# volume-em/empanada-napari

Measured on AMD Instinct MI355X. Metric: EM tiles/sec (1024^2 fp16), higher is better.
Workload: dtype f16

## Files before the change

### empanada-napari_amd/build.py

```python
import os
import shutil
import subprocess
import sys

HERE = os.path.dirname(os.path.abspath(__file__))
CSRC = os.path.join(HERE, 'csrc')
OBJ = os.path.join(CSRC, '_obj')
LIBDIR = os.path.join(HERE, 'lib')
LIB = os.path.join(LIBDIR, 'libempanada_hip.so')
ARCH = 'gfx950'

COMMON = ['--offload-arch=' + ARCH, '-O3', '-std=c++17', '-fPIC', '-fvisibility=hidden',
          '-Wall', '-Wno-unused-function', '-Wno-unused-result']
PER_FILE = {
    'postprocess.hip': ['-ffp-contract=off', '-fhip-fp32-correctly-rounded-divide-sqrt'],
    'pdl_net.hip': ['-std=c++20'],
    'pdl_net32.hip': ['-std=c++20'],
}
SOURCES = ['abi.hip', 'conv_igemm.hip', 'layers.hip', 'pointrend.hip', 'postprocess.hip', 'pdl_net.hip', 'pdl_net32.hip', 'sparse.hip',
           'sepconv.hip', 'sepconv_precise.hip', 'conv_igemm256.hip', 'conv_igemm_s64.hip', 'conv3x3c64.hip', 'stem.hip', 'matcher.hip', 'ref32.hip', 'conv16x3.hip', 'conv_igemm_grouped.hip', 'conv16x3p.hip', 'sepconv_x3.hip', 'overlap.hip', 'labels.hip', 'measure.hip', 'morph.hip', 'split.hip']
INCLUDES = {'conv_igemm_grouped.hip': ['conv_igemm.hip']}


def _hipcc():
    for cand in (shutil.which('hipcc'), '/opt/rocm/bin/hipcc'):
        if cand and os.path.exists(cand):
            return cand
    raise RuntimeError('hipcc not found: the HIP engine cannot be built (no CPU fallback exists)')


def _newest_header():
    hs = [os.path.join(CSRC, f) for f in os.listdir(CSRC) if f.endswith('.h')]
    hs.append(os.path.join(HERE, '..', 'include', 'empanada_hip.h'))
    return max(os.path.getmtime(h) for h in hs)


def build_all(verbose=False, force=False):
    os.makedirs(OBJ, exist_ok=True)
    os.makedirs(LIBDIR, exist_ok=True)
    hipcc = _hipcc()
    hdr = _newest_header()
    objs, rebuilt = [], False
    procs = []
    for src in SOURCES:
        s = os.path.join(CSRC, src)
        o = os.path.join(OBJ, src.replace('.hip', '.o'))
        objs.append(o)
        dep = max([os.path.getmtime(s), hdr] + [os.path.getmtime(os.path.join(CSRC, d)) for d in INCLUDES.get(src, [])])
        if force or not os.path.exists(o) or os.path.getmtime(o) < dep:
            cmd = [hipcc] + COMMON + PER_FILE.get(src, []) + ['-c', s, '-o', o]
            if verbose:
                print(' '.join(cmd), flush=True)
            procs.append((src, subprocess.Popen(cmd, stdout=subprocess.PIPE, stderr=subprocess.STDOUT)))
            rebuilt = True
    for src, p in procs:
        out, _ = p.communicate()
        if p.returncode != 0:
            sys.stderr.write(out.decode())
            raise RuntimeError(f'hipcc failed on {src}')
        if verbose and out.strip():
            print(out.decode())
    if rebuilt or not os.path.exists(LIB):
        cmd = [hipcc, '--offload-arch=' + ARCH, '-shared', '-fPIC', '-o', LIB] + objs
        if verbose:
            print(' '.join(cmd), flush=True)
        subprocess.check_call(cmd)
    return LIB


if __name__ == '__main__':
    print(build_all(verbose=True, force='--force' in sys.argv))
```

### empanada-napari_amd/csrc/abi.hip

```cpp
#include <stdarg.h>

#include <map>
#include <mutex>
#include <utility>
#include <vector>

#include "common.h"

namespace emp {

static thread_local char g_err[1024] = "no error";

void set_error(const char* fmt, ...) {
  va_list ap;
  va_start(ap, fmt);
  vsnprintf(g_err, sizeof(g_err), fmt, ap);
  va_end(ap);
}

const void* zero_page() {
  static void* page = nullptr;
  static std::once_flag once;
  std::call_once(once, [] {
    if (hipMalloc(&page, 2048) != hipSuccess) { page = nullptr; return; }
    if (hipMemset(page, 0, 2048) != hipSuccess) { (void)hipFree(page); page = nullptr; }
  });
  return page;
}

int ensure_dyn_lds(const void* kernel, int bytes) {
  static std::mutex mu;
  static std::map<std::pair<int, const void*>, int> done;
  int dev = 0;
  EMP_CHECK_HIP(hipGetDevice(&dev));
  std::lock_guard<std::mutex> lk(mu);
  auto it = done.find({dev, kernel});
  if (it != done.end() && it->second >= bytes) return EMP_OK;
  EMP_CHECK_HIP(hipFuncSetAttribute(kernel, hipFuncAttributeMaxDynamicSharedMemorySize, bytes));
  done[{dev, kernel}] = bytes;
  return EMP_OK;
}

}

using namespace emp;

extern "C" {

const char* emp_last_error(void) { return g_err; }
int emp_abi_version(void) { return 5; }

int emp_device_count(void) {
  int n = 0;
  hipError_t e = hipGetDeviceCount(&n);
  if (e != hipSuccess) {
    set_error("hipGetDeviceCount: %s", hipGetErrorString(e));
    return EMP_ERR_HIP;
  }
  return n;
}

int emp_copy_d2d(void* d_dst, const void* d_src, size_t bytes, void* stream) {
  EMP_REQUIRE(d_dst && d_src, "copy_d2d: null pointer");
  EMP_CHECK_HIP(hipMemcpyAsync(d_dst, d_src, bytes, hipMemcpyDeviceToDevice, (hipStream_t)stream));
  return EMP_OK;
}

int emp_conv2d_nhwc_f16(const void* d_in, int N, int H, int W, int Cin, int in_ld, const void* d_w,
                        const float* d_bias, const float* d_bias_n, const void* d_res, int res_ld, void* d_out,
                        int out_ld, int Cout, int KH, int KW, int stride, int pad, int dil, int relu, int variant,
                        void* stream) {
  EMP_REQUIRE(d_in && d_w && d_out, "conv2d: null pointer");
  EMP_REQUIRE(N > 0 && H > 0 && W > 0 && KH > 0 && KW > 0 && stride > 0 && dil > 0 && pad >= 0, "conv2d: bad geometry");
  EMP_REQUIRE(variant >= 0 && (variant & 15) <= 3 && ((variant >> 4) & 15) <= 7 && ((variant >> 8) & 255) <= 64 && (variant >> 16) <= 31, "conv2d: bad variant %d", variant);
  ConvParams p{};
  p.in = (const half_t*)d_in;
  p.wgt = (const half_t*)d_w;
  p.bias = d_bias;
  p.bias_n = d_bias_n;
  p.res = (const half_t*)d_res;
  p.res_ld = res_ld;
  p.out = (half_t*)d_out;
  p.zero = (const half_t*)zero_page();
  EMP_REQUIRE(p.zero != nullptr, "conv2d: could not allocate the zero page");
  p.N = N; p.H = H; p.W = W; p.Cin = Cin; p.in_ld = in_ld;
  p.Cout = Cout; p.KH = KH; p.KW = KW; p.stride = stride; p.pad = pad; p.dil = dil;
  p.Ho = (H + 2 * pad - dil * (KH - 1) - 1) / stride + 1;
  p.Wo = (W + 2 * pad - dil * (KW - 1) - 1) / stride + 1;
  EMP_REQUIRE(p.Ho > 0 && p.Wo > 0, "conv2d: empty output");
  p.out_ld = out_ld;
  p.act = relu;
  p.ps_cout = 0;
  p.M = N * p.Ho * p.Wo;
  return launch_conv_igemm(p, variant, (hipStream_t)stream);
}

int emp_conv256_pack_weights(const void* d_w, void* d_packed, int Cout, int KT, int Cin, int Cin2, void* stream) {
  return conv256_pack_weights((const half_t*)d_w, (half_t*)d_packed, Cout, KT, Cin, Cin2, (hipStream_t)stream);
}

int emp_conv2d_nhwc_f32(const float* d_in, int N, int H, int W, int Cin, int in_ld, const float* d_w, const float* d_bias,
                        const float* d_bias_n, const float* d_res, int res_ld, float* d_out, int out_ld, int Cout, int KH,
                        int KW, int stride, int pad, int dil, int act, void* stream) {
  EMP_REQUIRE(d_in && d_w && d_out, "conv2d_f32: null pointer");
  EMP_REQUIRE(N > 0 && H > 0 && W > 0 && KH > 0 && KW > 0 && stride > 0 && dil > 0 && pad >= 0, "conv2d_f32: bad geometry");
  Conv32 p{};
  p.in = d_in; p.in_ld = in_ld; p.w = d_w; p.bias = d_bias; p.bias_n = d_bias_n; p.res = d_res; p.res_ld = res_ld;
  p.out = d_out; p.out_ld = out_ld;
  p.N = N; p.H = H; p.W = W; p.Cin = Cin; p.Cout = Cout; p.KH = KH; p.KW = KW; p.stride = stride; p.pad = pad; p.dil = dil;
  p.Ho = (H + 2 * pad - dil * (KH - 1) - 1) / stride + 1;
  p.Wo = (W + 2 * pad - dil * (KW - 1) - 1) / stride + 1;
  EMP_REQUIRE(p.Ho > 0 && p.Wo > 0 && out_ld >= Cout && (d_res == nullptr || res_ld >= Cout), "conv2d_f32: bad output geometry");
  p.act = act;
  return launch_conv32(p, (hipStream_t)stream);
}

int emp_conv2d_nhwc_f16x3(const float* d_in, int N, int H, int W, int Cin, int in_ld, const float* d_w, const float* d_bias,
                          const float* d_bias_n, const float* d_res, int res_ld, float* d_out, int out_ld, int Cout, int KH,
                          int KW, int stride, int pad, int dil, int act, int groups, int cin_g, void* stream) {
  EMP_REQUIRE(d_in && d_w && d_out, "conv2d_f16x3: null pointer");
  EMP_REQUIRE(N > 0 && H > 0 && W > 0 && KH > 0 && KW > 0 && stride > 0 && dil > 0 && pad >= 0 && groups >= 1, "conv2d_f16x3: bad geometry");
  Conv32 p{};
  p.in = d_in; p.in_ld = in_ld; p.w = d_w; p.bias = d_bias; p.bias_n = d_bias_n; p.res = d_res; p.res_ld = res_ld;
  p.out = d_out; p.out_ld = out_ld;
  p.N = N; p.H = H; p.W = W; p.Cin = Cin; p.Cout = Cout; p.KH = KH; p.KW = KW; p.stride = stride; p.pad = pad; p.dil = dil;
  p.Ho = (H + 2 * pad - dil * (KH - 1) - 1) / stride + 1;
  p.Wo = (W + 2 * pad - dil * (KW - 1) - 1) / stride + 1;
  EMP_REQUIRE(p.Ho > 0 && p.Wo > 0 && out_ld >= groups * Cout && (d_res == nullptr || res_ld >= Cout), "conv2d_f16x3: bad output geometry");
  p.act = act;
  p.x3 = 1;
  if (groups > 1) { p.groups = groups; p.cin_g = cin_g; }
  return launch_conv32(p, (hipStream_t)stream);
}

int emp_conv2d_nhwc_f16x3_ex(const float* d_in, int N, int H, int W, int Cin, int in_ld, const float* d_w, const float* d_bias,
                             const float* d_bias_n, const float* d_res, int res_ld, void* d_out, int out_ld, int out_fmt, int Cout, int KH,
                             int KW, int stride, int pad, int dil, int act, int wmode, const float* d_in2, int H2, int W2, int Cin2,
                             int in2_ld, int stride2, const float* d_head_w, const float* d_head_b, int head_c, float* d_head_out,
                             void* stream) {
  EMP_REQUIRE(d_in && d_w && (d_out || d_head_w), "conv2d_f16x3_ex: null pointer");
  EMP_REQUIRE(N > 0 && H > 0 && W > 0 && KH > 0 && KW > 0 && stride > 0 && dil > 0 && pad >= 0 && wmode >= 0 && (wmode & 3) <= 2 && wmode < 8,
              "conv2d_f16x3_ex: bad geometry (wmode 0 fp32 weights, 1 split pairs, 2 pairs + LDS-DMA image; + 4: split-K allowed)");
  const bool ksplit = (wmode & 4) != 0;
  wmode &= 3;
  hipStream_t s = (hipStream_t)stream;
  Conv32 p{};
  p.in = d_in; p.in_ld = in_ld; p.w = d_w; p.bias = d_bias; p.bias_n = d_bias_n; p.res = d_res; p.res_ld = res_ld;
  p.out = (float*)d_out; p.out_ld = out_ld; p.out_fmt = out_fmt;
  p.N = N; p.H = H; p.W = W; p.Cin = Cin; p.Cout = Cout; p.KH = KH; p.KW = KW; p.stride = stride; p.pad = pad; p.dil = dil;
  p.Ho = (H + 2 * pad - dil * (KH - 1) - 1) / stride + 1;
  p.Wo = (W + 2 * pad - dil * (KW - 1) - 1) / stride + 1;
  EMP_REQUIRE(p.Ho > 0 && p.Wo > 0 && (d_head_w || out_ld >= Cout) && (d_res == nullptr || res_ld >= Cout), "conv2d_f16x3_ex: bad output geometry");
  p.act = act;
  p.x3 = 1;
  if (d_in2) { p.in2 = d_in2; p.in2_ld = in2_ld; p.Cin2 = Cin2; p.H2 = H2; p.W2 = W2; p.stride2 = stride2; }
  const int64_t Krow = (int64_t)KH * KW * Cin + (d_in2 ? Cin2 : 0);
  std::vector<void*> tmp;
  auto cleanup = [&]() { for (void* q : tmp) (void)hipFree(q); };
  int rc = EMP_OK;
  if (wmode >= 1) {
    void* d = nullptr;
    if (hipMalloc(&d, (size_t)Cout * Krow * sizeof(uint32_t)) != hipSuccess) { cleanup(); set_error("conv2d_f16x3_ex: out of memory"); return EMP_ERR_NOMEM; }
    tmp.push_back(d);
    p.wpair = (const uint32_t*)d;
    rc = launch_split_pairs(d_w, (uint32_t*)d, (int64_t)Cout * Krow, s);
  }
  if (!rc && wmode == 2 && !d_in2) {
    const int64_t ih = x3_weight_image_halfs(Cout, (int)Krow, Cin);
    if (ih > 0) {
      void* d = nullptr;
      if (hipMalloc(&d, (size_t)ih * sizeof(half_t)) != hipSuccess) { cleanup(); set_error("conv2d_f16x3_ex: out of memory"); return EMP_ERR_NOMEM; }
      tmp.push_back(d);
      p.wimg = (const half_t*)d;
      rc = launch_x3_weight_image(d_w, (half_t*)d, Cout, (int)Krow, s);
    }
  }
  if (!rc && ksplit && !d_head_w && !d_in2) {
    void* d = nullptr;
    if (hipMalloc(&d, (size_t)X3_KPART_BYTES) != hipSuccess) { cleanup(); set_error("conv2d_f16x3_ex: out of memory"); return EMP_ERR_NOMEM; }
    tmp.push_back(d);
    p.kpart = (float*)d; p.kpart_bytes = X3_KPART_BYTES;
  }
  const int64_t MP = (int64_t)N * p.Ho * p.Wo;
  const int tiles = conv16x3_cout_tiles(Cout);
  if (!rc && d_head_w) {
    EMP_REQUIRE(d_head_out && head_c >= 1 && head_c <= 4, "conv2d_f16x3_ex: the fused head writes (N, head_c, Ho * Wo) floats, head_c <= 4");
    void* d = nullptr;
    if (hipMalloc(&d, (size_t)tiles * MP * head_c * sizeof(float)) != hipSuccess) { cleanup(); set_error("conv2d_f16x3_ex: out of memory"); return EMP_ERR_NOMEM; }
    tmp.push_back(d);
    p.head_w = d_head_w; p.head_part = (float*)d; p.head_c = head_c;
    if (!p.out) { p.out = d_head_out; p.out_ld = Cout; }
  }
  if (!rc) rc = launch_conv32(p, s);
  if (!rc && d_head_w) rc = launch_head_finish_f32(p.head_part, tiles, N, p.Ho * p.Wo, head_c, d_head_b, d_head_out, s);
  hipError_t e = hipStreamSynchronize(s);
  cleanup();
  if (!rc && e != hipSuccess) { set_error("conv2d_f16x3_ex: %s", hipGetErrorString(e)); return EMP_ERR_HIP; }
  return rc;
}

int emp_sepconv_x3_pack(const float* d_dw, const float* d_pw, int ks, int C, int Cout, float* d_dw_packed, void* d_pw_packed, void* stream) {
  int rc = launch_sepx3_pack_dw(d_dw, ks, C, C, d_dw_packed, (hipStream_t)stream);
  if (rc) return rc;
  return launch_sepx3_pack_pw(d_pw, C, C, Cout, (half_t*)d_pw_packed, (hipStream_t)stream);
}
int emp_sepconv_x3_nhwc_f32(const float* d_in, int N, int H, int W, int C, int in_ld, const float* d_dw_packed, const void* d_pw_packed,
                            const float* d_bias, int Cout, int act, float* d_out, int out_ld, const float* d_head_w, const float* d_head_b,
                            int head_c, float* d_head_out, int ks, void* stream) {
  EMP_REQUIRE(N > 0 && H > 0 && W > 0, "sepconv_x3: bad geometry");
  return launch_sepconv_x3(d_in, N, H, W, C, in_ld, d_dw_packed, (const half_t*)d_pw_packed, d_bias, Cout, act, d_out, out_ld, d_head_w,
                           d_head_b, head_c, d_head_out, (int64_t)H * W, (hipStream_t)stream, ks);
}

int emp_hl32_from_f32(const float* d_in, void* d_out, int64_t rows, int C, int in_ld, int out_ld, void* stream) {
  return launch_hl32_from_f32(d_in, (half_t*)d_out, rows, C, in_ld, out_ld, (hipStream_t)stream);
}
int emp_hl32_to_f32(const void* d_in, float* d_out, int64_t rows, int C, int in_ld, int out_ld, void* stream) {
  return launch_hl32_to_f32((const half_t*)d_in, d_out, rows, C, in_ld, out_ld, (hipStream_t)stream);
}
int emp_x3p_pack_weights(const float* d_w, void* d_img, int Cout, int K, void* stream) {
  return launch_x3p_pack(d_w, (half_t*)d_img, Cout, K, (hipStream_t)stream);
}
int emp_conv2d_hl32_f16x3(const void* d_in, int N, int H, int W, int Cin, int in_ld, const void* d_wimg, const float* d_bias,
                          const float* d_bias_n, const void* d_res, int res_ld, int res_fmt, void* d_out, int out_ld, int out_fmt,
                          int Cout, int KH, int KW, int stride, int pad, int dil, int act, void* stream) {
  EMP_REQUIRE(d_in && d_wimg && d_out, "conv2d_hl32_f16x3: null pointer");
  EMP_REQUIRE(N > 0 && H > 0 && W > 0 && KH > 0 && KW > 0 && stride > 0 && dil > 0 && pad >= 0, "conv2d_hl32_f16x3: bad geometry");
// ... 337 lines not shown
```

### empanada-napari_amd/csrc/common.h

```cpp
#pragma once
#include <hip/hip_runtime.h>
#include <stdint.h>
#include <stdio.h>
#include <stdlib.h>
#include <string>

#include "../../include/empanada_hip.h"

typedef _Float16 half_t;
typedef _Float16 f16x8 __attribute__((ext_vector_type(8)));
typedef _Float16 f16x4 __attribute__((ext_vector_type(4)));
typedef _Float16 f16x2 __attribute__((ext_vector_type(2)));
typedef float f32x4 __attribute__((ext_vector_type(4)));

namespace emp {

void set_error(const char* fmt, ...);

#define EMP_CHECK_HIP(expr)                                                        \
  do {                                                                             \
    hipError_t _e = (expr);                                                        \
    if (_e != hipSuccess) {                                                        \
      emp::set_error("%s:%d: %s -> %s", __FILE__, __LINE__, #expr, hipGetErrorString(_e)); \
      return EMP_ERR_HIP;                                                          \
    }                                                                              \
  } while (0)

#define EMP_REQUIRE(cond, ...)          \
  do {                                  \
    if (!(cond)) {                      \
      emp::set_error(__VA_ARGS__);      \
      return EMP_ERR_INVALID;           \
    }                                   \
  } while (0)

#define EMP_LAUNCH_CHECK() EMP_CHECK_HIP(hipGetLastError())

const void* zero_page();

int ensure_dyn_lds(const void* kernel, int bytes);

static inline int cdiv(int a, int b) { return (a + b - 1) / b; }
static inline int64_t cdiv64(int64_t a, int64_t b) { return (a + b - 1) / b; }

static inline bool env_on(const char* name) { const char* e = getenv(name); return !(e && e[0] == '0'); }
static inline int env_int(const char* name, int dflt) { const char* e = getenv(name); return e ? atoi(e) : dflt; }
static inline int64_t env_i64(const char* name, int64_t dflt) { const char* e = getenv(name); return e ? atoll(e) : dflt; }

struct ConvParams {
  const half_t* in;
  const half_t* wgt;
  const float* bias;
  const float* bias_n;
  const half_t* res;
  half_t* out;
  const half_t* zero;
  int N, H, W, Cin, in_ld;
  int Cout, KH, KW, stride, pad, dil;
  int Ho, Wo, out_ld, res_ld;
  int act;
  int ps_cout;
  int M;
  int mt, nt;
  int mt_per_xcd;
  int kgroup;
  int ngroup;
  const half_t* in2;
  int Cin2, in2_ld, H2, W2, stride2;
  half_t* out2;
  int out2_ld, split;
  half_t* out3;
  int out3_ld, split3;
  const half_t* next_w;
  const float* next_b;
  half_t* next_out;
  int next_cout, next_ld;
};

int launch_conv_igemm(const ConvParams& p, int variant, hipStream_t stream);
int launch_conv_igemm_grouped(const ConvParams& p, int groups, int gs_in, long long gs_w, int gs_out, hipStream_t stream);
bool conv_igemm256_supported(const ConvParams& p);
bool conv_uses_256(const ConvParams& p);
int launch_conv_igemm256(ConvParams p, hipStream_t stream, int kg = 0, int mode = 0, bool wpacked = false);
int conv256_pack_kgroup(int KT, int Cin);
int conv256_pack_weights(const half_t* w, half_t* out, int Cout, int KT, int Cin, int Cin2, hipStream_t stream);
bool conv_b2b_supported(const ConvParams& p);
bool conv_igemm_h256_supported(const ConvParams& p);
int launch_conv_igemm_h256(ConvParams p, hipStream_t stream, int kg = 0);
bool conv_igemm_s64_supported(const ConvParams& p);
int launch_conv_igemm_s64(ConvParams p, hipStream_t stream, int kg = 0);
bool conv3x3_c64_supported(const ConvParams& p);
int launch_conv3x3_c64(const ConvParams& p, hipStream_t stream);

int launch_stem7x7(const void* img, int dtype, float sub, float mul, int N, int H, int W, int vh, int vw,
                   const float* w , const float* b , half_t* out, hipStream_t s);
int launch_maxpool3x3s2(const half_t* in, int N, int H, int W, int C, half_t* out, hipStream_t s);
int launch_stem3x3s2_f16(const void* img, int dtype, float sub, float mul, int N, int H, int W, int vh, int vw,
                         const float* w , const float* b, int C, half_t* out, int out_ld, hipStream_t s);
int launch_gate_mul_f16(const half_t* x, int x_ld, half_t* g , int g_ld, int64_t rows, int C,
                        hipStream_t s);
int launch_stem_pool(const void* img, int dtype, float sub, float mul, int N, int H, int W, int vh, int vw,
                     const float* w, const float* b, half_t* out, hipStream_t s);
int launch_stem_pool_f32(const void* img, int dtype, float sub, float mul, int N, int H, int W, int vh, int vw,
                         const float* w, const float* b, float* out, hipStream_t s);
int launch_dwconv(const half_t* in, int N, int H, int W, int C, int in_ld, const half_t* w, int K,
                  half_t* out, int out_ld, const half_t* zero, hipStream_t s);
int launch_fuse_combine(const half_t* a, const half_t* b, const half_t* c, float ca, float cb, float cc, int mode,
                        int N, int H, int W, int C, half_t* out, hipStream_t s, half_t* out_lo = nullptr, int out_ld = 0);
int launch_bilinear_ac(const half_t* in, int N, int h, int w, int C, int in_ld, half_t* out, int H, int W,
                       int out_ld, hipStream_t s, int variant = 0);
int launch_avgpool(const half_t* in, int N, int HW, int C, int in_ld, float* out , float* part,
                   hipStream_t s);
int avgpool_scratch_floats(int N, int C);
int launch_gemv(const float* in, int N, int K, const float* w, const float* b, int Cout, int relu,
                float* out, hipStream_t s);
bool sepconv5_supported(int C, int Cout, int head_c);
int launch_sepconv5_pack_pw(const half_t* w, int pw_ld, int C, int Cout, half_t* packed, hipStream_t s);
int launch_sepconv5(const half_t* in, int N, int H, int W, int C, int in_ld, const half_t* dww, const half_t* pww_packed,
                    const float* bias, int Cout, int act, half_t* out, int out_ld, const float* head_w,
                    const float* head_b, int head_c, float* hout, int64_t plane, const half_t* zero, hipStream_t s,
                    int ks = 5);
bool sepconvp_supported(int C, int Cout, int head_c);
bool sepconvp_wsplit_supported(int Cout);
int launch_sepconvp_pack_pw(const float* w, int pw_ld, int C, int Cout, half_t* packed, hipStream_t s, int wsplit = 0);
int launch_sepconvp_pack_dw(const float* w, int ks, int C, float* packed, hipStream_t s);
int launch_sepconvp(const half_t* in, int N, int H, int W, int C, int in_ld, const float* dww_packed, const half_t* pww_packed,
                    const float* bias, int Cout, int act, half_t* out, int out_ld, const float* head_w,
                    const float* head_b, int head_c, float* hout, int64_t plane, const half_t* zero, hipStream_t s,
                    int ks = 5, int wsplit = 0);
int launch_head1x1(const half_t* in, int N, int P, int K, int in_ld, const float* w, const float* b, int C,
                   float* out, int64_t plane_size, const int32_t* scatter_idx, hipStream_t s);
int launch_bilinear_ac_f32_nchw(const float* in, int NC, int h, int w, float* out, int scale, hipStream_t s);
int launch_zero(void* p, size_t bytes, hipStream_t s);

struct Conv32 {
  const float* in; int in_ld;
  const float* w; const float* bias; const float* bias_n;
  const float* res; int res_ld;
  float* out; int out_ld;
  int N, H, W, Cin, Cout, KH, KW, stride, pad, dil, Ho, Wo;
  int act;
  int ps_cout;
  int groups;
  int cin_g;
  int x3;
  const float* in2; int in2_ld, Cin2, H2, W2, stride2;
  const float* head_w; float* head_part; int head_c;
  int x3_mt, x3_nt, x3_mtx;
  const float* zero;
  const uint32_t* wpair;
  const half_t* wimg;
  int in_fmt, out_fmt, res_fmt;
  const half_t* wimgp;
  float* out2; int out2_ld, split2;
  int x3p_kg;
  float* kpart; int64_t kpart_bytes; int ksplit, x3_ksteps;
};
constexpr int64_t X3_KPART_BYTES = 64ll << 20;
int launch_conv32(const Conv32& p, hipStream_t s);
int launch_conv16x3(const Conv32& p, hipStream_t s);
int launch_split_pairs(const float* w, uint32_t* out, int64_t n, hipStream_t s);
int64_t x3_weight_image_halfs(int Cout, int K, int Cin);
int launch_x3_weight_image(const float* w, half_t* out, int Cout, int K, hipStream_t s);
bool conv16x3p_supported(const Conv32& p);
int launch_conv16x3p(const Conv32& p, hipStream_t s);
int64_t x3p_image_halfs(int Cout, int K);
int x3p_kgroup(int KT, int Cin);
int launch_x3p_pack(const float* w, half_t* out, int Cout, int K, hipStream_t s, int KT = 0, int Cin = 0, int kg = 0);
int launch_hl32_from_f32(const float* in, half_t* out, int64_t rows, int C, int in_ld, int out_ld, hipStream_t s);
int launch_hl32_to_f32(const half_t* in, float* out, int64_t rows, int C, int in_ld, int out_ld, hipStream_t s);
int launch_avgpool_hl32(const half_t* in, int N, int HW, int C, int in_ld, float* out, hipStream_t s);
bool sepconv_x3_supported(int C, int Cout, int head_c, int ks);
int64_t sepx3_pw_halfs(int C, int Cout);
int launch_sepx3_pack_pw(const float* w, int pw_ld, int C, int Cout, half_t* packed, hipStream_t s);
int launch_sepx3_pack_dw(const float* w , int ks, int C, int ld, float* packed, hipStream_t s);
int launch_sepconv_x3(const float* in, int N, int H, int W, int C, int in_ld, const float* dww, const half_t* pww, const float* bias,
                      int Cout, int act, float* out, int out_ld, const float* head_w, const float* head_b, int head_c, float* hout,
                      int64_t plane, hipStream_t s, int ks = 5);
int conv16x3_cout_tiles(int Cout);
int launch_head_finish_f32(const float* part, int tiles, int N, int P, int C, const float* b, float* out, hipStream_t s);
int launch_stem3x3s2_f32(const void* img, int dtype, float sub, float mul, int N, int H, int W, int vh, int vw,
                         const float* w , const float* b, int C, float* out, int out_ld, hipStream_t s);
int launch_gate_mul_f32(float* x, int x_ld, const float* g, int g_ld, int64_t rows, int C, hipStream_t s);
int launch_stem7x7_f32(const void* img, int dtype, float sub, float mul, int N, int H, int W, int vh, int vw,
                       const float* w , const float* b , float* out, hipStream_t s);
int launch_maxpool3x3s2_f32(const float* in, int N, int H, int W, int C, float* out, hipStream_t s);
int launch_dwconv_f32(const float* in, int N, int H, int W, int C, int in_ld, const float* w , int K, float* out,
                      int out_ld, hipStream_t s);
int launch_bilinear_ac_f32_nhwc(const float* in, int N, int h, int w, int C, int in_ld, float* out, int H, int W, int out_ld,
                                hipStream_t s);
int launch_avgpool_f32(const float* in, int N, int HW, int C, int in_ld, float* out, hipStream_t s);
int launch_fuse_combine_f32(const float* a, const float* b, const float* c, float ca, float cb, float cc, int mode, int N,
                            int H, int W, int C, float* out, hipStream_t s);
int launch_head1x1_f32(const float* in, int N, int P, int K, int in_ld, const float* w, const float* b, int C, float* out,
                       int64_t plane_size, const int32_t* scatter_idx, hipStream_t s);
int launch_point_features_f32(const float* feat, int N, int fh, int fw, int C, int feat_ld, const float* coarse, int ncls,
                              const int32_t* idx, int P, int H2, int W2, float* x0, float* x1, int ld, hipStream_t s);

size_t topk_work_bytes(int N, int64_t plane);
int launch_upsample2x_keys(const float* in, int N, int C, int h, int w, float* out, uint32_t* keys, hipStream_t s);
int launch_topk_smallest(const uint32_t* keys, int N, int64_t plane, int k, void* work, size_t work_bytes,
                         int32_t* idx_out, hipStream_t s);
int launch_point_features(const half_t* feat, int N, int fh, int fw, int C, int feat_ld, const float* coarse,
                          int ncls, const int32_t* idx, int P, int H2, int W2, half_t* x0, half_t* x1, int ld,
                          hipStream_t s);

__device__ __forceinline__ float pr_sample_pos(int i, int grid, int size) {
#pragma clang fp contract(off)
  const float step = 1.0f / (float)grid;
  const float c = 0.5f * step + step * (float)i;
  const float g = 2.0f * c - 1.0f;
  return ((g + 1.f) * (float)size - 1.f) * 0.5f;
}

bool pr_mlp_supported(int C, int ld, int ncls, int num_fc);
int launch_pr_mlp(const half_t* feat, int N, int fh, int fw, int C, int feat_ld, const float* coarse, int ncls,
                  const int32_t* idx, int P, int H2, int W2, const half_t* const* fc_w, const float* const* fc_b,
                  int num_fc, int ld, const float* pred_w, const float* pred_b, float* out, int64_t plane, hipStream_t s);


}
```

### empanada-napari_amd/csrc/conv_igemm.hip

```cpp
#include "igemm_common.h"

#ifdef EMP_IGEMM_GROUPED
#define EMP_IGEMM_KARGS const ConvParams p_, const int gs_in, const long long gs_w, const int gs_out
#define EMP_IGEMM_KPROLOGUE                                                \
  ConvParams p = p_;                                                       \
  {                                                                        \
    const int g_ = blockIdx.y;                                             \
    p.in += (size_t)g_ * gs_in;                                            \
    p.wgt += (size_t)g_ * (size_t)gs_w;                                    \
    p.out += (size_t)g_ * gs_out;                                          \
    if (p.bias) p.bias += (size_t)g_ * gs_out;                             \
  }
#else
#define EMP_IGEMM_KARGS const ConvParams p
#define EMP_IGEMM_KPROLOGUE
#endif

#include <type_traits>

namespace emp {

namespace {

constexpr int BK = 64;
// ... 250 lines not shown
    constexpr int RB = TN * 4;
    constexpr int C4 = TN / 4;
    static_assert(4 * TM * RB <= 2 * (A_BYTES + B_BYTES), "staging tile must fit the main-loop LDS");
    char* stg = lds + w * (TM * RB);
#pragma unroll
    for (int t = 0; t < PT; ++t) {
      const int row = t * 16 + fr;
#pragma unroll
      for (int c = 0; c < CT; ++c) {
        const int ch = (c >> 1) * 8 + fq * 2 + (c & 1);
        *reinterpret_cast<f32x4*>(stg + row * RB + ((ch ^ (row & (C4 - 1))) << 4)) = acc[c][t];
      }
    }
    __builtin_amdgcn_s_waitcnt(0xc07f);
    dispatch_act(p.act, [&](auto act_tag) __attribute__((always_inline)) {
    constexpr int ACT = decltype(act_tag)::value;
#pragma unroll
    for (int i = 0; i < TM / RPI; ++i) {
      const int row = i * RPI + l / CPR;
      const int m = m0 + wm * TM + row;
      const f32x4 a0 = *reinterpret_cast<const f32x4*>(stg + row * RB + (((2 * c8) ^ (row & (C4 - 1))) << 4));
      const f32x4 a1 = *reinterpret_cast<const f32x4*>(stg + row * RB + (((2 * c8 + 1) ^ (row & (C4 - 1))) << 4));
      float v[8];
#pragma unroll
      for (int r = 0; r < 4; ++r) { v[r] = a0[r] + bv[r]; v[4 + r] = a1[r] + bv[4 + r]; }
      if (m >= p.M || !co_ok) continue;
      if (p.bias_n) {
        const float* bn = p.bias_n + (size_t)(m / HoWo) * p.Cout + co_l;
        const float4 b0 = *reinterpret_cast<const float4*>(bn);
        const float4 b1 = *reinterpret_cast<const float4*>(bn + 4);
        v[0] += b0.x; v[1] += b0.y; v[2] += b0.z; v[3] += b0.w;
        v[4] += b1.x; v[5] += b1.y; v[6] += b1.z; v[7] += b1.w;
      }
      if (p.res) {
#pragma unroll
        for (int r = 0; r < 8; ++r) v[r] += (float)rres[i][r];
      }
      f16x8 o;
#pragma unroll
      for (int r = 0; r < 8; ++r) o[r] = (half_t)conv_act<ACT>(v[r]);
      *reinterpret_cast<f16x8*>(out_ptr(p, m, co_l, HoWo)) = o;
    }
    });
    return;
  } else {
    compute((S - 1) & 1);
    dispatch_act(p.act, [&](auto act_tag) __attribute__((always_inline)) {
    constexpr int ACT = decltype(act_tag)::value;
#pragma unroll
    for (int t = 0; t < PT; ++t) {
      const int m = m0 + wm * TM + t * 16 + fr;
      if (m >= p.M) continue;
      const int n_img = (p.bias_n != nullptr) ? m / HoWo : 0;
#pragma unroll
      for (int P = 0; P < CT / 2; ++P) {
        const int co = n0 + wn * TN + P * 32 + fq * 8;
        if (co >= p.Cout) continue;
        float v[8];
#pragma unroll
        for (int r = 0; r < 4; ++r) {
          v[r] = acc[2 * P][t][r];
          v[4 + r] = acc[2 * P + 1][t][r];
        }
        if (p.bias) {
          const float4 b0 = *reinterpret_cast<const float4*>(p.bias + co);
          const float4 b1 = *reinterpret_cast<const float4*>(p.bias + co + 4);
          v[0] += b0.x; v[1] += b0.y; v[2] += b0.z; v[3] += b0.w;
          v[4] += b1.x; v[5] += b1.y; v[6] += b1.z; v[7] += b1.w;
        }
        if (p.bias_n) {
          const float* bn = p.bias_n + (size_t)n_img * p.Cout + co;
          const float4 b0 = *reinterpret_cast<const float4*>(bn);
          const float4 b1 = *reinterpret_cast<const float4*>(bn + 4);
          v[0] += b0.x; v[1] += b0.y; v[2] += b0.z; v[3] += b0.w;
          v[4] += b1.x; v[5] += b1.y; v[6] += b1.z; v[7] += b1.w;
        }
        if (p.res) {
          const f16x8 rv = *reinterpret_cast<const f16x8*>(p.res + (size_t)m * p.res_ld + co);
#pragma unroll
          for (int r = 0; r < 8; ++r) v[r] += (float)rv[r];
        }
        f16x8 o;
#pragma unroll
        for (int r = 0; r < 8; ++r) o[r] = (half_t)conv_act<ACT>(v[r]);
        *reinterpret_cast<f16x8*>(out_ptr(p, m, co, HoWo)) = o;
      }
    }
    });
  }
}

#ifdef EMP_IGEMM_GROUPED
template <int BM, int BN, int WPM, int WPN, bool GLDS, bool EPI_LDS, int OCC = 2>
int launch_grouped_tpl(ConvParams p, int groups, int gs_in, long long gs_w, int gs_out, hipStream_t stream) {
  const int grid = fill_raster(p, BM, BN);
  hipLaunchKernelGGL((conv_igemm_kernel<BM, BN, WPM, WPN, GLDS, EPI_LDS, OCC>), dim3(grid, groups), dim3(256), 0, stream, p, gs_in,
                     gs_w, gs_out);
  EMP_LAUNCH_CHECK();
  return EMP_OK;
}

}

int launch_conv_igemm_grouped(const ConvParams& p, int groups, int gs_in, long long gs_w, int gs_out, hipStream_t stream) {
  EMP_REQUIRE(groups >= 1 && groups < 65536, "grouped conv: bad group count %d", groups);
  EMP_REQUIRE(p.Cin % BK == 0 && p.Cin > 0 && p.in_ld % 8 == 0 && (groups - 1) * gs_in + p.Cin <= p.in_ld && gs_in % 8 == 0,
              "grouped conv: Cin=%d (multiple of 64), channel step %d (multiple of 8), row %d", p.Cin, gs_in, p.in_ld);
  EMP_REQUIRE(p.Cout % 8 == 0 && p.Cout > 0 && gs_out % 8 == 0 && gs_out >= p.Cout && p.out_ld % 8 == 0 &&
                  (groups - 1) * gs_out + p.Cout <= p.out_ld, "grouped conv: Cout=%d, cout step %d, row %d", p.Cout, gs_out, p.out_ld);
  EMP_REQUIRE(gs_w % 8 == 0 && gs_w >= (long long)p.Cout * p.KH * p.KW * p.Cin, "grouped conv: weight stride %lld", gs_w);
  EMP_REQUIRE(!p.in2 && !p.out2 && !p.out3 && !p.next_w && !p.res && !p.bias_n && p.ps_cout == 0, "grouped conv: plain convolutions only");
  EMP_REQUIRE(p.act >= 0 && p.act <= 2, "grouped conv: act must be 0, 1 or 2");
  EMP_REQUIRE(((uintptr_t)p.in % 16) == 0 && ((uintptr_t)p.out % 16) == 0 && ((uintptr_t)p.wgt % 16) == 0 &&
                  ((uintptr_t)p.zero % 256) == 0 && p.zero != nullptr, "grouped conv: pointers must be 16-byte aligned (zero page 256)");
  EMP_REQUIRE((int64_t)p.N * p.Ho * p.Wo < (1ll << 31), "grouped conv: too many output pixels");
  ConvParams q = p;
  {
    const int CB = p.Cin / 64, KT = p.KH * p.KW;
    int kg = (KT > 1 && CB > 4 && CB % 4 == 0) ? 4 : CB;
    q.kgroup = kg;
  }
  if (p.Cout <= 64 || cdiv(p.Cout, 64) * 64 <= cdiv(p.Cout, 128) * 128)
    return launch_grouped_tpl<128, 64, 2, 2, true, true, 3>(q, groups, gs_in, gs_w, gs_out, stream);
  return launch_grouped_tpl<128, 128, 2, 2, true, true>(q, groups, gs_in, gs_w, gs_out, stream);
}

#else
template <int BM, int BN, int WPM, int WPN, bool GLDS, bool EPI_LDS, int OCC = 2>
int launch_tpl(ConvParams p, hipStream_t stream) {
  const int grid = fill_raster(p, BM, BN);
  hipLaunchKernelGGL((conv_igemm_kernel<BM, BN, WPM, WPN, GLDS, EPI_LDS, OCC>), dim3(grid), dim3(256), 0, stream, p);
  EMP_LAUNCH_CHECK();
  return EMP_OK;
}

}

bool conv_uses_256(const ConvParams& p) {
  static const bool no256 = env_is("EMP_CONV_NO256", '1');
  static const int min_k = env_int("EMP_CONV_256_MINK", 512);
  const int64_t tiles256 = (int64_t)cdiv(p.M, 256) * (p.Cout / 256);
  const int k256 = p.KH * p.KW * p.Cin + (p.in2 ? p.Cin2 : 0);
  const bool out2_ok = !p.out2 || (!p.out3 && p.split % 256 == 0);
  return !no256 && out2_ok && conv_igemm256_supported(p) && tiles256 >= 192 && k256 >= (p.in2 ? min_k / 4 : min_k);
}
bool conv_uses_h256(const ConvParams& p) {
  static const int h256 = env_int("EMP_CONV_H256", 1);
  if (!h256 || !conv_igemm_h256_supported(p)) return false;
  const int64_t tiles = (int64_t)cdiv(p.M, 128) * (p.Cout / 128) / 2;
  if (tiles < 1024) return false;
  return h256 == 2 || (p.Cout == 128 && p.KH * p.KW * p.Cin >= 256);
}

int launch_conv_igemm(const ConvParams& p, int variant, hipStream_t stream) {
  EMP_REQUIRE(p.Cin % BK == 0 && p.Cin > 0, "conv: Cin=%d must be a positive multiple of 64", p.Cin);
  EMP_REQUIRE(p.in_ld % 8 == 0 && p.in_ld >= p.Cin, "conv: in_ld=%d must be >= Cin and a multiple of 8", p.in_ld);
  EMP_REQUIRE(p.Cout % 8 == 0 && p.Cout > 0, "conv: Cout=%d must be a positive multiple of 8", p.Cout);
  EMP_REQUIRE(p.out_ld % 8 == 0 && p.out_ld >= (p.ps_cout ? p.ps_cout : (p.out2 ? p.split : p.Cout)), "conv: out_ld=%d invalid", p.out_ld);
  EMP_REQUIRE(p.ps_cout == 0 || (p.ps_cout % 8 == 0 && p.Cout == 4 * p.ps_cout && p.res == nullptr),
              "conv: pixel-shuffle store needs Cout == 4*ps_cout, ps_cout %% 8 == 0, no residual");
  EMP_REQUIRE(p.act >= 0 && p.act <= 2, "conv: act must be 0 (none), 1 (ReLU) or 2 (SiLU)");
  EMP_REQUIRE(p.res == nullptr || p.res_ld % 8 == 0, "conv: res_ld=%d must be a multiple of 8", p.res_ld);
  EMP_REQUIRE(((uintptr_t)p.in % 16) == 0 && ((uintptr_t)p.out % 16) == 0 && ((uintptr_t)p.wgt % 16) == 0 &&
                  ((uintptr_t)p.res % 16) == 0 && ((uintptr_t)p.zero % 256) == 0 && p.zero != nullptr,
              "conv: pointers must be 16-byte aligned (zero page 256)");
  EMP_REQUIRE((int64_t)p.N * p.Ho * p.Wo < (1ll << 31), "conv: too many output pixels");
  if (p.out2) {
    EMP_REQUIRE(p.split > 0 && p.split < p.Cout && p.split % 8 == 0 && p.out2_ld % 8 == 0 &&
                    p.out2_ld >= (p.out3 ? p.split3 : p.Cout) - p.split &&
                    p.out_ld >= p.split && ((uintptr_t)p.out2 % 16) == 0 && p.ps_cout == 0 && p.res == nullptr,
                "conv: second destination: split=%d must be a multiple of 8 inside (0, Cout=%d)", p.split, p.Cout);
  }
  if (p.out3) {
    EMP_REQUIRE(p.out2 != nullptr && p.split3 > p.split && p.split3 < p.Cout && p.split3 % 8 == 0 && p.out3_ld % 8 == 0 &&
                    p.out3_ld >= p.Cout - p.split3 && ((uintptr_t)p.out3 % 16) == 0,
                "conv: third destination: split3=%d must be a multiple of 8 inside (split=%d, Cout=%d)", p.split3, p.split, p.Cout);
  }
  if (p.in2) {
    EMP_REQUIRE(p.KH == 1 && p.KW == 1 && p.stride == 1 && p.pad == 0,
                "conv: a second source needs a 1x1 / stride 1 main convolution");
    EMP_REQUIRE(p.Cin2 > 0 && p.Cin2 % BK == 0 && p.in2_ld % 8 == 0 && p.in2_ld >= p.Cin2 && ((uintptr_t)p.in2 % 16) == 0,
                "conv: second source: Cin2=%d must be a positive multiple of 64, in2_ld=%d >= Cin2", p.Cin2, p.in2_ld);
    EMP_REQUIRE(p.stride2 >= 1 && (p.Ho - 1) * p.stride2 < p.H2 && (p.Wo - 1) * p.stride2 < p.W2,
                "conv: second source %dx%d / stride %d does not cover the %dx%d output", p.H2, p.W2, p.stride2, p.Ho, p.Wo);
  }
  int v = variant & 15, tile = (variant >> 4) & 15, kg = (variant >> 8) & 255, mode256 = (variant >> 16) & 15;
  if ((variant >> 20) & 1) {
    EMP_REQUIRE(!p.next_w && conv_igemm256_supported(p), "conv: packed weights belong to the 256x256 tile");
    return launch_conv_igemm256(p, stream, 0, mode256, true);
  }
  if (p.next_w) {
    EMP_REQUIRE(conv_b2b_supported(p), "conv: a fused next convolution needs the 256x256 tile (Cout == 256, >= 192 tiles)");
    return launch_conv_igemm256(p, stream, kg, mode256);
  }
  EMP_REQUIRE(v <= 3 && tile <= 7, "conv: bad variant %d", variant);
  if (tile == 7) return launch_conv_igemm_s64(p, stream, kg);
  if (tile == 6) return launch_conv3x3_c64(p, stream);
  if (tile == 5) return launch_conv_igemm_h256(p, stream, kg);
  {
    static const bool no_c64 = env_is("EMP_CONV_NO_C64", '1');
    if (tile == 0 && !no_c64 && conv3x3_c64_supported(p) && (int64_t)p.N * cdiv(p.H, 8) * cdiv(p.W, 16) >= 1024)
      return launch_conv3x3_c64(p, stream);
  }
  if (tile == 4) {
    return launch_conv_igemm256(p, stream, kg, mode256);
  }
  ConvParams q = p;
  {
    const int CB = p.Cin / 64, KT = p.KH * p.KW;
    static const int env_kg = env_int("EMP_CONV_KGROUP", 0);
    if (kg == 0) kg = env_kg;
    if (kg == 0) kg = (KT > 1 && CB > 4 && CB % 4 == 0) ? 4 : CB;
    if (kg > CB || CB % kg != 0 || KT == 1) kg = CB;
    q.kgroup = kg;
  }
  if (tile == 0) {
    if (conv_uses_256(p)) return launch_conv_igemm256(p, stream);
    if (conv_uses_h256(p)) return launch_conv_igemm_h256(p, stream);
    tile = (p.Cout <= 64) ? 2 : 1;
    if (p.Cout > 128 && cdiv(p.Cout, 64) * 64 < cdiv(p.Cout, 128) * 128) tile = 2;
    static const int small_below = env_int("EMP_CONV_SMALL_TILES_BELOW", 256);
    if (tile == 1 && (int64_t)cdiv(p.M, 128) * cdiv(p.Cout, 128) < small_below && !p.out2) {
      static const bool no_s64 = env_is("EMP_CONV_NO_S64", '1');
      if (!no_s64 && conv_igemm_s64_supported(p)) return launch_conv_igemm_s64(p, stream);
      tile = 3;
    }
  }
  if (v == 0) v = 3;
  if (tile == 1) {
    if (v == 1) return launch_tpl<128, 128, 2, 2, false, false>(q, stream);
    if (v == 2) return launch_tpl<128, 128, 2, 2, true, false>(q, stream);
    return launch_tpl<128, 128, 2, 2, true, true>(q, stream);
  }
  if (tile == 2) {
    if (v == 1) return launch_tpl<128, 64, 2, 2, false, false, 3>(q, stream);
    if (v == 2) return launch_tpl<128, 64, 2, 2, true, false, 3>(q, stream);
    return launch_tpl<128, 64, 2, 2, true, true, 3>(q, stream);
  }
  if (v == 1) return launch_tpl<64, 64, 2, 2, false, false, 5>(q, stream);
  if (v == 2) return launch_tpl<64, 64, 2, 2, true, false, 5>(q, stream);
  return launch_tpl<64, 64, 2, 2, true, true, 5>(q, stream);
}

#endif

}
```

Before: 1386.

## Add persistent register-weight 1x1 conv kernel with triple-buffered LDS DMA ring

Adds a persistent 1x1 convolution kernel for 256- or 512-channel inputs with small output widths. Each wave holds its slice of the weights in registers, and pixel tiles stream through a three-slot LDS ring filled by async DMA loads with counted waits. It is selected automatically for large enough problems unless an environment variable disables it. In exchange it adds a large register footprint (launch bounds 512,1) and a new code path with odd-row-tile shuffles that could mis-store if wrong.

```diff
diff --git a/empanada-napari_amd/build.py b/empanada-napari_amd/build.py
--- a/empanada-napari_amd/build.py
+++ b/empanada-napari_amd/build.py
@@ -18,7 +18,7 @@
     'pdl_net32.hip': ['-std=c++20'],
 }
 SOURCES = ['abi.hip', 'conv_igemm.hip', 'layers.hip', 'pointrend.hip', 'postprocess.hip', 'pdl_net.hip', 'pdl_net32.hip', 'sparse.hip',
-           'sepconv.hip', 'sepconv_precise.hip', 'conv_igemm256.hip', 'conv_igemm_s64.hip', 'conv3x3c64.hip', 'stem.hip', 'matcher.hip', 'ref32.hip', 'conv16x3.hip', 'conv_igemm_grouped.hip', 'conv16x3p.hip', 'sepconv_x3.hip', 'overlap.hip', 'labels.hip', 'measure.hip', 'morph.hip', 'split.hip']
+           'sepconv.hip', 'sepconv_precise.hip', 'conv_igemm256.hip', 'conv_igemm_s64.hip', 'conv3x3c64.hip', 'conv1x1rw.hip', 'stem.hip', 'matcher.hip', 'ref32.hip', 'conv16x3.hip', 'conv_igemm_grouped.hip', 'conv16x3p.hip', 'sepconv_x3.hip', 'overlap.hip', 'labels.hip', 'measure.hip', 'morph.hip', 'split.hip']
 INCLUDES = {'conv_igemm_grouped.hip': ['conv_igemm.hip']}
 
 
diff --git a/empanada-napari_amd/csrc/abi.hip b/empanada-napari_amd/csrc/abi.hip
--- a/empanada-napari_amd/csrc/abi.hip
+++ b/empanada-napari_amd/csrc/abi.hip
@@ -72,7 +72,7 @@
                         void* stream) {
   EMP_REQUIRE(d_in && d_w && d_out, "conv2d: null pointer");
   EMP_REQUIRE(N > 0 && H > 0 && W > 0 && KH > 0 && KW > 0 && stride > 0 && dil > 0 && pad >= 0, "conv2d: bad geometry");
-  EMP_REQUIRE(variant >= 0 && (variant & 15) <= 3 && ((variant >> 4) & 15) <= 7 && ((variant >> 8) & 255) <= 64 && (variant >> 16) <= 31, "conv2d: bad variant %d", variant);
+  EMP_REQUIRE(variant >= 0 && (variant & 15) <= 3 && ((variant >> 4) & 15) <= 8 && ((variant >> 8) & 255) <= 64 && (variant >> 16) <= 31, "conv2d: bad variant %d", variant);
   ConvParams p{};
   p.in = (const half_t*)d_in;
   p.wgt = (const half_t*)d_w;
diff --git a/empanada-napari_amd/csrc/common.h b/empanada-napari_amd/csrc/common.h
--- a/empanada-napari_amd/csrc/common.h
+++ b/empanada-napari_amd/csrc/common.h
@@ -91,6 +91,9 @@
 int launch_conv_igemm_s64(ConvParams p, hipStream_t stream, int kg = 0);
 bool conv3x3_c64_supported(const ConvParams& p);
 int launch_conv3x3_c64(const ConvParams& p, hipStream_t stream);
+bool conv1x1_rw_supported(const ConvParams& p);
+int conv1x1_rw_tiles(const ConvParams& p);
+int launch_conv1x1_rw(const ConvParams& p, hipStream_t stream);
 
 int launch_stem7x7(const void* img, int dtype, float sub, float mul, int N, int H, int W, int vh, int vw,
                    const float* w , const float* b , half_t* out, hipStream_t s);
diff --git a/empanada-napari_amd/csrc/conv1x1rw.hip b/empanada-napari_amd/csrc/conv1x1rw.hip
--- /dev/null
+++ b/empanada-napari_amd/csrc/conv1x1rw.hip
@@ -0,0 +1,216 @@
+#include "igemm_common.h"
+
+namespace emp {
+namespace {
+
+constexpr int RW_SLOT = 32 * 1024;
+constexpr int RW_RING = 3;
+constexpr int RW_NDMA = 4;
+constexpr int RW_CG = 4, RW_PG = 2;
+
+struct Rw1x1Params {
+  const half_t* in;
+  const half_t* wgt;
+  const float* bias;
+  half_t* out;
+  half_t* out2;
+  half_t* out3;
+  const half_t* zero;
+  int M, Cout, in_ld, out_ld, out2_ld, out3_ld, split, split3;
+  int tiles;
+};
+
+template <int CIN, int NRT, int PT, int ACT>
+__global__ void __launch_bounds__(512, 1) conv1x1_rw_kernel(const Rw1x1Params p) {
+  constexpr int KS = CIN / 32;
+  constexpr int ROWB = CIN * 2;
+  constexpr int TP = RW_PG * PT * 16;
+  constexpr int LPP = ROWB / 16;
+  constexpr int PPP = 64 / LPP;
+  constexpr int CPW = NRT * 16;
+  constexpr int NPAIR = NRT / 2;
+  static_assert(TP * ROWB == RW_SLOT && RW_NDMA * 8 * 1024 == RW_SLOT, "a tile is 32 pieces");
+  static_assert(RW_NDMA == 4 && RW_RING == 3, "the counted waits below say vmcnt(4), the slot walk is modulo 3");
+  static_assert(NRT % 2 == 0 || PT % 2 == 0, "the odd row tile trades halves between two pixel tiles");
+  extern __shared__ __attribute__((aligned(1024))) char lds[];
+  const int tid = threadIdx.x, lane = tid & 63;
+  const int wave = __builtin_amdgcn_readfirstlane(tid >> 6);
+  const int pg = wave >> 2, cg = wave & 3;
+  const int fr = lane & 15, fq = lane >> 4;
+
+  const int xcd = blockIdx.x & 7, jx = blockIdx.x >> 3, nx = gridDim.x >> 3;
+  auto tile_of = [&](int it) { return (it * 8 + xcd) * nx + jx; };
+  int my_tiles = 0;
+  while (tile_of(my_tiles) < p.tiles) ++my_tiles;
+
+  f16x8 wreg[NRT][KS];
+#pragma unroll
+  for (int j = 0; j < NRT; ++j) {
+    const int row = j < 2 * NPAIR ? (j & ~1) * 16 + perm32((j & 1) * 16 + fr) : j * 16 + fr;
+    const int co = cg * CPW + row;
+    const half_t* wr = p.wgt + (size_t)co * CIN + fq * 8;
+    if (co < p.Cout) {
+#pragma unroll
+      for (int s = 0; s < KS; ++s) wreg[j][s] = *reinterpret_cast<const f16x8*>(wr + s * 32);
+    } else {
+#pragma unroll
+      for (int s = 0; s < KS; ++s) wreg[j][s] = f16x8{0, 0, 0, 0, 0, 0, 0, 0};
+    }
+  }
+  auto dest = [&](int co, half_t*& d, int& ld) {
+    d = nullptr;
+    ld = 0;
+    if (co >= p.Cout) return;
+    if (co >= p.split3) { d = p.out3 + (co - p.split3); ld = p.out3_ld; }
+    else if (co >= p.split) { d = p.out2 + (co - p.split); ld = p.out2_ld; }
+    else { d = p.out + co; ld = p.out_ld; }
+  };
+  float bvp[NPAIR > 0 ? NPAIR : 1][8];
+  half_t* dp[NPAIR > 0 ? NPAIR : 1];
+  int dld[NPAIR > 0 ? NPAIR : 1];
+#pragma unroll
+  for (int P = 0; P < NPAIR; ++P) {
+    const int co = cg * CPW + P * 32 + fq * 8;
+#pragma unroll
+    for (int r = 0; r < 8; ++r) bvp[P][r] = (p.bias && co < p.Cout) ? p.bias[co + r] : 0.f;
+    dest(co, dp[P], dld[P]);
+  }
+  float bvo[4] = {0.f, 0.f, 0.f, 0.f};
+  half_t* dpo = nullptr;
+  int dldo = 0;
+  if constexpr (NRT % 2 == 1) {
+    const int co = cg * CPW + (NRT - 1) * 16 + fq * 4;
+#pragma unroll
+    for (int r = 0; r < 4; ++r) bvo[r] = (p.bias && co < p.Cout) ? p.bias[co + r] : 0.f;
+    dest(cg * CPW + (NRT - 1) * 16 + (fq & ~1) * 4, dpo, dldo);
+  }
+  asm volatile("s_waitcnt vmcnt(0)" ::: "memory");
+
+  auto stage = [&](int it, int slot) {
+    const bool valid = it < my_tiles;
+    const int m0 = valid ? tile_of(it) * TP : 0;
+    char* sb = lds + slot * RW_SLOT;
+#pragma unroll
+    for (int k = 0; k < RW_NDMA; ++k) {
+      const int piece = wave + 8 * k;
+      const int px = piece * PPP + lane / LPP;
+      const int m = m0 + px;
+      const bool ok = valid && m < p.M;
+      const half_t* src = ok ? p.in + (size_t)m * p.in_ld + (((lane % LPP) ^ (px & 15)) << 3) : p.zero;
+      lds_dma16(src, sb + piece * 1024);
+    }
+  };
+
+  int pf_off[PT][4];
+#pragma unroll
+  for (int t = 0; t < PT; ++t)
+#pragma unroll
+    for (int q = 0; q < 4; ++q) pf_off[t][q] = ((pg * PT + t) * 16 + fr) * ROWB + (((fq ^ fr) ^ (q << 2)) << 4);
+
+  stage(0, 0);
+  stage(1, 1);
+  asm volatile("s_waitcnt vmcnt(4)" ::: "memory");
+  lds_barrier();
+
+  int slot = 0;
+  for (int it = 0; it < my_tiles; ++it) {
+    stage(it + 2, slot == 0 ? 2 : slot - 1);
+    const char* sb = lds + slot * RW_SLOT;
+    f32x4 acc[NRT][PT];
+#pragma unroll
+    for (int j = 0; j < NRT; ++j)
+#pragma unroll
+      for (int t = 0; t < PT; ++t) acc[j][t] = f32x4{0.f, 0.f, 0.f, 0.f};
+#pragma unroll
+    for (int s = 0; s < KS; ++s) {
+      f16x8 pf[PT];
+#pragma unroll
+      for (int t = 0; t < PT; ++t) pf[t] = *reinterpret_cast<const f16x8*>(sb + pf_off[t][s & 3] + (s >> 2) * 256);
+#pragma unroll
+      for (int j = 0; j < NRT; ++j)
+#pragma unroll
+        for (int t = 0; t < PT; ++t) acc[j][t] = __builtin_amdgcn_mfma_f32_16x16x32_f16(wreg[j][s], pf[t], acc[j][t], 0, 0, 0);
+    }
+    asm volatile("s_waitcnt vmcnt(4)" ::: "memory");
+    {
+      const int mb = tile_of(it) * TP + pg * PT * 16 + fr;
+#pragma unroll
+      for (int t = 0; t < PT; ++t) {
+        const int m = mb + t * 16;
+#pragma unroll
+        for (int P = 0; P < NPAIR; ++P) {
+          f16x8 o;
+#pragma unroll
+          for (int r4 = 0; r4 < 4; ++r4) {
+            o[r4] = (half_t)conv_act<ACT>(acc[2 * P][t][r4] + bvp[P][r4]);
+            o[4 + r4] = (half_t)conv_act<ACT>(acc[2 * P + 1][t][r4] + bvp[P][4 + r4]);
+          }
+          if (m < p.M && dp[P]) *reinterpret_cast<f16x8*>(dp[P] + (size_t)m * dld[P]) = o;
+        }
+      }
+      if constexpr (NRT % 2 == 1) {
+        const int odd = fq & 1;
+#pragma unroll
+        for (int t2 = 0; t2 < PT / 2; ++t2) {
+          typedef _Float16 f16x4 __attribute__((ext_vector_type(4)));
+          typedef int i32x2 __attribute__((ext_vector_type(2)));
+          f16x4 h[2];
+#pragma unroll
+          for (int u = 0; u < 2; ++u)
+#pragma unroll
+            for (int r4 = 0; r4 < 4; ++r4) h[u][r4] = (half_t)conv_act<ACT>(acc[NRT - 1][2 * t2 + u][r4] + bvo[r4]);
+          const i32x2 a0 = __builtin_bit_cast(i32x2, h[0]), a1 = __builtin_bit_cast(i32x2, h[1]);
+          const i32x2 keep = odd ? a1 : a0, send = odd ? a0 : a1;
+          i32x2 recv;
+          recv[0] = __shfl_xor(send[0], 16);
+          recv[1] = __shfl_xor(send[1], 16);
+          typedef int i32x4 __attribute__((ext_vector_type(4)));
+          const i32x4 o = odd ? i32x4{recv[0], recv[1], keep[0], keep[1]} : i32x4{keep[0], keep[1], recv[0], recv[1]};
+          const int m = mb + (2 * t2 + odd) * 16;
+          if (m < p.M && dpo) *reinterpret_cast<i32x4*>(dpo + (size_t)m * dldo) = o;
+        }
+      }
+    }
+    lds_barrier();
+    slot = slot == 2 ? 0 : slot + 1;
+  }
+  asm volatile("s_waitcnt vmcnt(0)" ::: "memory");
+}
+
+template <int CIN, int NRT, int PT>
+int launch_rw(const Rw1x1Params& p, int act, int grid, hipStream_t stream) {
+  auto go = [&](auto kern) -> int { return launch_dyn(kern, grid, 512, RW_RING * RW_SLOT, stream, p); };
+  if (act == 1) return go(&conv1x1_rw_kernel<CIN, NRT, PT, 1>);
+  if (act == 2) return go(&conv1x1_rw_kernel<CIN, NRT, PT, 2>);
+  return go(&conv1x1_rw_kernel<CIN, NRT, PT, 0>);
+}
+
+}
+
+bool conv1x1_rw_supported(const ConvParams& p) {
+  return ((p.Cin == 256 && p.Cout <= 192) || (p.Cin == 512 && p.Cout <= 128)) && p.KH == 1 && p.KW == 1 && p.stride == 1 && p.pad == 0 &&
+         p.res == nullptr && p.bias_n == nullptr && p.ps_cout == 0 && p.in2 == nullptr && p.next_w == nullptr &&
+         p.M <= (1 << 30);
+}
+int conv1x1_rw_tiles(const ConvParams& p) { return cdiv(p.M, p.Cin == 256 ? 64 : 32); }
+
+int launch_conv1x1_rw(const ConvParams& q, hipStream_t stream) {
+  EMP_REQUIRE(conv1x1_rw_supported(q), "conv1x1_rw: unsupported shape (1x1 / stride 1, 256 -> <= 192 or 512 -> <= 128 channels, no residual, "
+                                       "per-image bias, second source, pixel shuffle or fused next convolution)");
+  Rw1x1Params p{};
+  p.in = q.in; p.wgt = q.wgt; p.bias = q.bias; p.zero = q.zero;
+  p.out = q.out; p.out2 = q.out2; p.out3 = q.out3;
+  p.M = q.M; p.Cout = q.Cout; p.in_ld = q.in_ld; p.out_ld = q.out_ld; p.out2_ld = q.out2_ld; p.out3_ld = q.out3_ld;
+  p.split3 = q.out3 ? q.split3 : q.Cout;
+  p.split = q.out2 ? q.split : p.split3;
+  p.tiles = conv1x1_rw_tiles(q);
+  int grid = 256;
+  while (grid > 8 && grid > p.tiles) grid -= 8;
+  const int cap = env_int("EMP_CONV_RW1X1_GRID", 0);
+  if (cap > 0 && cap < grid) grid = cap < 8 ? 8 : cap & ~7;
+  if (q.Cin == 512) return launch_rw<512, 2, 1>(p, q.act, grid, stream);
+  if (q.Cout <= 128) return launch_rw<256, 2, 2>(p, q.act, grid, stream);
+  return launch_rw<256, 3, 2>(p, q.act, grid, stream);
+}
+
+}
diff --git a/empanada-napari_amd/csrc/conv_igemm.hip b/empanada-napari_amd/csrc/conv_igemm.hip
--- a/empanada-napari_amd/csrc/conv_igemm.hip
+++ b/empanada-napari_amd/csrc/conv_igemm.hip
@@ -426,6 +426,13 @@
   return h256 == 2 || (p.Cout == 128 && p.KH * p.KW * p.Cin >= 256);
 }
 
+bool conv1x1_rw_uses(const ConvParams& p) {
+  if (!conv1x1_rw_supported(p) || env_is("EMP_CONV_NO_RW1X1", '1')) return false;
+  if (!(p.Cout == 128 || (p.Cin == 256 && p.Cout > 128))) return false;
+  const int dflt = p.Cin == 512 ? 8192 : (p.Cout > 128 ? 1024 : 2048);
+  return conv1x1_rw_tiles(p) >= env_int("EMP_CONV_RW1X1_MIN_TILES", dflt);
+}
+
 int launch_conv_igemm(const ConvParams& p, int variant, hipStream_t stream) {
   EMP_REQUIRE(p.Cin % BK == 0 && p.Cin > 0, "conv: Cin=%d must be a positive multiple of 64", p.Cin);
   EMP_REQUIRE(p.in_ld % 8 == 0 && p.in_ld >= p.Cin, "conv: in_ld=%d must be >= Cin and a multiple of 8", p.in_ld);
@@ -467,7 +474,8 @@
     EMP_REQUIRE(conv_b2b_supported(p), "conv: a fused next convolution needs the 256x256 tile (Cout == 256, >= 192 tiles)");
     return launch_conv_igemm256(p, stream, kg, mode256);
   }
-  EMP_REQUIRE(v <= 3 && tile <= 7, "conv: bad variant %d", variant);
+  EMP_REQUIRE(v <= 3 && tile <= 8, "conv: bad variant %d", variant);
+  if (tile == 8) return launch_conv1x1_rw(p, stream);
   if (tile == 7) return launch_conv_igemm_s64(p, stream, kg);
   if (tile == 6) return launch_conv3x3_c64(p, stream);
   if (tile == 5) return launch_conv_igemm_h256(p, stream, kg);
@@ -476,6 +484,7 @@
     if (tile == 0 && !no_c64 && conv3x3_c64_supported(p) && (int64_t)p.N * cdiv(p.H, 8) * cdiv(p.W, 16) >= 1024)
       return launch_conv3x3_c64(p, stream);
   }
+  if (tile == 0 && conv1x1_rw_uses(p)) return launch_conv1x1_rw(p, stream);
   if (tile == 4) {
     return launch_conv_igemm256(p, stream, kg, mode256);
   }
```

Result: no change. 1396 (median of 6 runs) (+0.7%).
